# mikelodder7/bls-bn254

Hardware: AMD Instinct MI355X
Metric: BN254 pairings/sec (= BLS verifies/sec) (higher is better)
Workload: dtype int64; 1 GPU; 262144 batched single-sig BLS verifies per GPU (BASELINE configs[1]), unique 32-byte messages, 1024-key pool, 1/64 invalid tuples; key de-duplication + hash-to-G1 + per-key G2 checks and line tables + 2-pair Miller loop + final exp; tuples_per_gpu=262144, tuples_total=262144, key_pool=1024

## Files before the change

### bls-bn254_amd/csrc/fp29.h

```cpp
#pragma once
#include <stdint.h>
#include "bn254_consts.h"

#if defined(__HIPCC__)
#include <hip/hip_runtime.h>
#define BN_HD __host__ __device__
#else
#define BN_HD
#endif
#define BN_INL BN_HD inline __attribute__((always_inline))
#ifdef BN_FORCE_INLINE
#define BN_FUNC BN_INL
#else
#define BN_FUNC BN_HD inline
#endif

#define BN_UNROLL _Pragma("unroll")
#if defined(__HIP_DEVICE_COMPILE__)
#define BN_SCHED_BARRIER __builtin_amdgcn_sched_barrier(0)
#else
#define BN_SCHED_BARRIER ((void)0)
#endif

#ifdef BN_CHECK
#include <cmath>
#include <cstdio>
#include <cstdlib>
#endif

namespace bn {

constexpr int NL = 9;
constexpr int RB = 29;
constexpr int32_t MASK = (1 << RB) - 1;

struct Fp {
  int32_t l[NL];
#ifdef BN_CHECK
  double lo = 0, hi = 0;
  double tlo = 0, thi = 0;
  double vb = 0;
#endif
};

#ifdef BN_CHECK
struct CheckStats { double worst_mul = 0, worst_dot = 0, worst_vb = 0; long muls = 0, sqrs = 0, dots = 0, norms = 0, lcs = 0, lc_terms = 0; };
inline CheckStats& check_stats() { static thread_local CheckStats s; return s; }
inline double mag(const Fp& a) { return std::fmax(std::fabs(a.lo), std::fabs(a.hi)); }
inline double tmag(const Fp& a) { return std::fmax(std::fabs(a.tlo), std::fabs(a.thi)); }
struct CtxStack { const char* name[64]; int line[64]; int n = 0; };
inline CtxStack& ctx_stack() { static thread_local CtxStack s; return s; }
struct CtxGuard {
  CtxGuard(const char* f, int l) { CtxStack& s = ctx_stack(); if (s.n < 64) { s.name[s.n] = f; s.line[s.n] = l; } ++s.n; }
  ~CtxGuard() { --ctx_stack().n; }
};
inline void check_fail(const char* what, double v) {
  std::fprintf(stderr, "BN_CHECK violation: %s (%g)\n  context:", what, v);
  CtxStack& s = ctx_stack();
  for (int i = 0; i < s.n && i < 64; ++i) std::fprintf(stderr, " > %s:%d", s.name[i], s.line[i]);
  std::fprintf(stderr, "\n");
  std::abort();
}
#define BN_CTX ::bn::CtxGuard _bn_ctx_guard(__func__, __LINE__)
inline void check_actual(const Fp& a, const char* where) {
  const double L = 536870912.0;
  for (int i = 0; i < NL; ++i) {
    double v = a.l[i] / L, lo = i == NL - 1 ? a.tlo : a.lo, hi = i == NL - 1 ? a.thi : a.hi;
    if (v < lo - 1e-6 || v > hi + 1e-6) { std::fprintf(stderr, "limb %d = %g outside [%g,%g] at %s\n", i, v, lo, hi, where); check_fail("actual limb outside proven interval", v); }
  }
// ... 473 lines not shown
```

### bls-bn254_amd/csrc/host.hip

```cpp
#include "host_common.h"

extern "C" {

const uint8_t NEG_G2_BYTES[128] = {
  0x19,0x8e,0x93,0x93,0x92,0x0d,0x48,0x3a,0x72,0x60,0xbf,0xb7,0x31,0xfb,0x5d,0x25,0xf1,0xaa,0x49,0x33,0x35,0xa9,0xe7,0x12,0x97,0xe4,0x85,0xb7,0xae,0xf3,0x12,0xc2,
  0x18,0x00,0xde,0xef,0x12,0x1f,0x1e,0x76,0x42,0x6a,0x00,0x66,0x5e,0x5c,0x44,0x79,0x67,0x43,0x22,0xd4,0xf7,0x5e,0xda,0xdd,0x46,0xde,0xbd,0x5c,0xd9,0x92,0xf6,0xed,
  0x27,0x5d,0xc4,0xa2,0x88,0xd1,0xaf,0xb3,0xcb,0xb1,0xac,0x09,0x18,0x75,0x24,0xc7,0xdb,0x36,0x39,0x5d,0xf7,0xbe,0x3b,0x99,0xe6,0x73,0xb1,0x3a,0x07,0x5a,0x65,0xec,
  0x1d,0x9b,0xef,0xcd,0x05,0xa5,0x32,0x3e,0x6d,0xa4,0xd4,0x35,0xf3,0xb6,0x17,0xcd,0xb3,0xaf,0x83,0x28,0x5c,0x2d,0xf7,0x11,0xef,0x39,0xc0,0x15,0x71,0x82,0x7f,0x9d};


const char* blsbn254_strerror(int code) {
  switch (code) {
    case 0: return "ok";
    case 1: return "invalid scalar bytes";
    case 2: return "invalid G1 bytes";
    case 3: return "invalid G2 bytes";
    case 4: return "invalid Gt bytes";
    case BLSBN254_ST_SHORT: return "too few usable partial signatures";
    case BLSBN254_E_ARG: return "invalid argument";
    case BLSBN254_E_HIP: return "HIP runtime error";
    case BLSBN254_E_NOMEM: return "out of device memory";
    case BLSBN254_E_NO_DEVICE: return "no gfx950 device available (there is no CPU fallback)";
    case BLSBN254_E_RCCL: return "RCCL error";
    default: return "unknown error";
// ... 8 lines not shown
  if (hipGetDeviceCount(&count) != hipSuccess || count <= 0 || device < 0 || device >= count) return BLSBN254_E_NO_DEVICE;
  hipDeviceProp_t prop;
  if (hipGetDeviceProperties(&prop, device) != hipSuccess) return BLSBN254_E_NO_DEVICE;
  if (std::strncmp(prop.gcnArchName, "gfx950", 6) != 0) return BLSBN254_E_NO_DEVICE;
  blsbn254_ctx* c = new blsbn254_ctx();
  c->device = device;
  if (const char* e = std::getenv("BLSBN254_CHUNK_LANES")) {
    size_t v = (size_t)std::strtoull(e, nullptr, 10) & ~(size_t)7;
    if (v >= 8 && v <= ((size_t)1 << 23)) c->chunk = v;
  }
  if (hipSetDevice(device) != hipSuccess || hipStreamCreateWithFlags(&c->stream, hipStreamNonBlocking) != hipSuccess) { delete c; return BLSBN254_E_HIP; }
  if (hipStreamCreateWithFlags(&c->stream2, hipStreamNonBlocking) != hipSuccess || hipEventCreateWithFlags(&c->ev_fork, hipEventDisableTiming) != hipSuccess ||
      hipEventCreateWithFlags(&c->ev_join, hipEventDisableTiming) != hipSuccess) { (void)hipStreamDestroy(c->stream); delete c; return BLSBN254_E_HIP; }
  if (getrandom(&c->kd_seed, sizeof c->kd_seed, 0) != (ssize_t)sizeof c->kd_seed) c->kd_seed = 0x5bd1e995u;
  if (const char* e = std::getenv("BLSBN254_AUTO_PREPARE")) c->auto_prepare = std::atoi(e) != 0;
  if (const char* e = std::getenv("BLSBN254_RLC_GROUP")) { long v = std::atol(e); if (v >= 2 && v <= 4096) { c->rlc_group = (size_t)v; c->rlc_group_auto = false; } }
  c->lanes_per_round = (size_t)prop.multiProcessorCount * 256;
  if (const char* e = std::getenv("BLSBN254_RLC_KEY_ROUND")) c->rlc_key_round = std::atoi(e) != 0;
  if (const char* e = std::getenv("BLSBN254_WIDE_FE")) c->wide_fe = std::atoi(e) != 0;
  if (const char* e = std::getenv("BLSBN254_ASYNC_VERIFY")) c->async_verify = std::atoi(e) != 0;
  if (const char* e = std::getenv("BLSBN254_KEY_CACHE")) { long v = std::atol(e); if (v >= 0 && v <= (long)PREP_MAX_KEYS) c->kc.max = (size_t)v; }
  if (const char* e = std::getenv("BLSBN254_QUAD_PREP")) c->quad_prep = std::atoi(e) != 0;
  if (const char* e = std::getenv("BLSBN254_SPLIT_EASY")) c->split_easy = std::atoi(e) != 0;
  c->tri_max = c->lanes_per_round / 4;
  if (const char* e = std::getenv("BLSBN254_TRI_MILLER")) c->tri_miller = std::atoi(e) != 0;
  if (const char* e = std::getenv("BLSBN254_TRI_FE")) c->tri_fe = std::atoi(e) != 0;
  if (const char* e = std::getenv("BLSBN254_TRI_MAX")) { long v = std::atol(e); if (v >= 0 && v <= (1 << 20)) c->tri_max = (size_t)v; }
  if (const char* e = std::getenv("BLSBN254_WIDE_FE_MAX")) { long v = std::atol(e); if (v >= 0 && v <= (1 << 20)) c->wide_fe_max = (size_t)v; }
  *out = c;
  return 0;
}
void blsbn254_ctx_destroy(blsbn254_ctx* c) {
  if (!c) return;
  (void)hipSetDevice(c->device);
  (void)hipStreamSynchronize(c->stream);
  (void)hipStreamSynchronize(c->stream2);
  for (auto& pv : c->pend) if (pv.ev) (void)hipEventDestroy(pv.ev);
  if (c->pend_host) (void)hipHostFree(c->pend_host);
  for (auto& kv : c->prof) for (auto& pr : kv.second.pending) { (void)hipEventDestroy(pr.first); (void)hipEventDestroy(pr.second); }
  (void)hipEventDestroy(c->ev_fork); (void)hipEventDestroy(c->ev_join);
  (void)hipStreamDestroy(c->stream2);
  (void)hipStreamDestroy(c->stream);
  delete c;
}
int blsbn254_ctx_synchronize(blsbn254_ctx* c) {
  if (!c) return BLSBN254_E_ARG;
// ... 101 lines not shown
  HIPCHK(c, hipMemcpyAsync(d, none, 4 * words, hipMemcpyHostToDevice, c->stream));
  return 0;
}
int min_index_read(blsbn254_ctx* c, const int* d, int* out) {
  TRY(download(c, out, d, 4));
  if (*out == NO_INDEX) *out = -1;
  return 0;
}
int first_bad(blsbn254_ctx* c, const uint8_t* d_status, size_t n, uint8_t mask, uint8_t val, int* out) {
  HIPCHK(c, c->misc.reserve(64));
  TRY(min_index_arm(c, (int*)c->misc.p, 1));
  TRY(launch(c, c->stream, "status_reduce", grid_lanes(n), k_status_reduce, d_status, n, mask, val, (int*)c->misc.p));
  return min_index_read(c, (const int*)c->misc.p, out);
}
int read_status(blsbn254_ctx* c, const uint8_t* d_status, int idx, uint8_t* st) { return download(c, st, d_status + idx, 1); }


int run_final_exp(blsbn254_ctx* c, int32_t* f, size_t n, size_t stride, int mode, const uint8_t* flags, const uint8_t* sub_ok,
                         uint8_t* d_bitmap, uint8_t* d_gt, int* d_is_one) {
  CHECK_LANES(c, stride);
  for (DevBuf& b : c->fe) HIPCHK(c, b.reserve(stride * 108 * 4));
  HIPCHK(c, c->fe_slots.reserve(stride * 108 * 4 * 10));
  int32_t* S = (int32_t*)c->fe_slots.p;
  int32_t *X = (int32_t*)c->fe[0].p, *A = (int32_t*)c->fe[1].p, *B = (int32_t*)c->fe[2].p, *C = (int32_t*)c->fe[3].p,
          *B2 = (int32_t*)c->fe[4].p, *D = (int32_t*)c->fe[5].p;
  if (n >= c->lanes_per_round / 2 && c->split_easy) {
    TRY(launch(c, c->stream, "fe_easy_head", grid_lanes(n), k_fe_easy_head, (const int32_t*)f, n, stride, A, B));
    TRY(launch(c, c->stream, "fe_inv4", grid_lanes((n + 3) / 4), k_fe_inv4, B, n, stride));
    TRY(launch(c, c->stream, "fe_easy_tail", grid_lanes(n), k_fe_easy_tail, (const int32_t*)f, f, n, stride, (const int32_t*)A, (const int32_t*)B));
  } else {
    TRY(launch(c, c->stream, "fe_easy", grid_lanes(n), k_fe_easy, (const int32_t*)f, f, n, stride));
  }
  if (c->wide_fe && n <= c->wide_fe_max) {
    uint8_t* one = nullptr;
    if (mode == 0) { HIPCHK(c, c->fe_wide_one.reserve(n)); one = (uint8_t*)c->fe_wide_one.p; }
    TRY(launch(c, c->stream, "fe_hard_wide", grid_wide(n), k_fe_hard_wide, (const int32_t*)f, n, stride, flags, sub_ok, one, d_gt, d_is_one, mode));
    if (mode == 0) TRY(launch(c, c->stream, "pack_bitmap", grid_lanes(n), k_pack_bitmap, (const uint8_t*)one, n, d_bitmap));
    return 0;
  }
  if (n <= c->tri_max && c->tri_fe) {
    HIPCHK(c, c->tri_vals.reserve(n * TRI_VALUE_LIMBS * 4));
    uint8_t* one = nullptr;
    if (mode == 0) { HIPCHK(c, c->fe_wide_one.reserve(n)); one = (uint8_t*)c->fe_wide_one.p; }
    TRY(launch(c, c->stream, "fe_tri_hard", grid_tri(n), k_fe_tri_hard, (const int32_t*)f, n, stride, (int32_t*)c->tri_vals.p, flags, sub_ok, one, d_gt, d_is_one, mode));
    if (mode == 0) TRY(launch(c, c->stream, "pack_bitmap", grid_lanes(n), k_pack_bitmap, (const uint8_t*)one, n, d_bitmap));
    return 0;
  }
  TRY(launch(c, c->stream, "fe_expx_h1", grid_lanes(n), k_fe_expx_h1, (const int32_t*)f, S, n, stride, A, B));
  TRY(launch(c, c->stream, "fe_expx_h2", grid_lanes(n), k_fe_expx_h2, (const int32_t*)B, S, n, stride, B, C, B2, D));
  TRY(launch(c, c->stream, "fe_expx", grid_lanes(n), k_fe_expx, (const int32_t*)D, X, S, n, stride));
  TRY(launch(c, c->stream, "fe_h3", grid_lanes(n), k_fe_h3, (const int32_t*)f, (const int32_t*)A, (const int32_t*)C, (const int32_t*)B2, (const int32_t*)X, S, n, stride,
             flags, sub_ok, d_bitmap, d_gt, d_is_one, mode));
  return 0;
}

int miller_to_ws(blsbn254_ctx* c, const uint8_t* d_g1, const uint8_t* d_g2, size_t n) {
  CHECK_LANES(c, n);
  HIPCHK(c, c->f_ws.reserve(n * 108 * 4));
  HIPCHK(c, c->status.reserve(n));
  if (c->wide_fe && n <= c->wide_fe_max / 2) {
    TRY(launch(c, c->stream, "miller_wide_1", grid_wide(n), k_miller_wide_1, d_g1, d_g2, n, (int32_t*)c->f_ws.p, n, (uint8_t*)c->status.p));
  } else if (n <= c->tri_max && c->tri_miller) {
    TRY(launch(c, c->stream, "miller_tri_1", grid_tri(n), k_miller_tri_1, d_g1, d_g2, n, (int32_t*)c->f_ws.p, n, (uint8_t*)c->status.p));
  } else {
    TRY(launch(c, c->stream, "miller_1", grid_lanes(n), k_miller_1, d_g1, d_g2, n, (int32_t*)c->f_ws.p, n, (uint8_t*)c->status.p));
  }
  return 0;
}
int decode_status_rc(blsbn254_ctx* c, const uint8_t* d_status, size_t n) {
  int bad;
  int rc = first_bad(c, d_status, n, 3, 3, &bad);
  if (rc) return rc;
  if (bad < 0) return 0;
  uint8_t st; rc = read_status(c, d_status, bad, &st);
  if (rc) return rc;
// ... 130 lines not shown
```

### bls-bn254_amd/csrc/host_common.h

```cpp
#pragma once
#include <hip/hip_runtime.h>
#include <sys/random.h>
#include <cstdio>
#include <cstdlib>
#include <cstring>
#include <algorithm>
#include <map>
#include <string>
#include <vector>

#include "sha256.h"
#include "lane_ops.h"
#include "kernels.h"
#include "key_cache.h"
#include "seg_plan.h"
#include "keyset_agg_plan.h"
#include "../../include/blsbn254.h"

using namespace bn;

#define BNH __attribute__((visibility("hidden")))

struct BNH DevBuf {
  void* p = nullptr; size_t cap = 0;
// ... 82 lines not shown
  uint32_t kd_seed = 0;
  bool auto_prepare = true;
  uint64_t stat_prepared_chunks = 0, stat_exact_chunks = 0, stat_grouped_aggregates = 0, stat_pairwise_aggregates = 0;
  DevBuf q_ws;
  DevBuf th_x, th_num, th_den, th_glv, th_part, th_part2;
  DevBuf fe_wide_one;
  bool wide_fe = true;
  size_t tri_max = 16384;
  bool tri_miller = true, tri_fe = true;
  DevBuf tri_vals;
  struct PendingVerify {
    bool active = false; const uint8_t *d_pks = nullptr, *d_msgs = nullptr, *d_sigs = nullptr; const uint64_t* d_off = nullptr;
    size_t n = 0; uint8_t* d_bitmap = nullptr; uint8_t dst[256]; size_t dst_len = 0; hipEvent_t ev = nullptr;
  } pend[4];
  int pend_head = 0, pend_count = 0;
  uint32_t* pend_host = nullptr;
  DevBuf pend_dev;
  size_t u_hint = 0;
  size_t u_max_seen = 0;
  bool async_verify = true;
  uint64_t stat_async_chunks = 0, stat_async_reruns = 0;
  bool quad_prep = true;
  bool split_easy = true;
  size_t wide_fe_max = 2048;
  DevBuf gs_items, gs_items_ok, gs_sum, gs_sum_ok, gs_pk;
  SegWs gs;
  DevBuf fe_slots;
  uint8_t dst_host[256];
  int dst_host_len = -1;
  size_t chunk = (size_t)1 << 22;
  MsmWs msm;
  PcWs pc;
  ThbWs thb;
  AgbWs agb;
  TdlWs tdl;
  TcWs tc;
  KsetWs kset;
  KaggWs kagg;
  uint64_t stat_kset[4] = {0, 0, 0, 0};
  uint64_t stat_kagg[4] = {0, 0, 0, 0};
  uint64_t stat_tc[4] = {0, 0, 0, 0};
  uint64_t stat_tdl[4] = {0, 0, 0, 0};
  uint64_t stat_agb[4] = {0, 0, 0, 0};
  uint64_t stat_thb[3] = {0, 0, 0};
  int msm_window = 0;
  uint64_t stat_msm[4] = {0, 0, 0, 0};
  bool profiling = false;
  std::map<std::string, ProfEntry> prof;
  std::string last_error;
// ... 152 lines not shown
```

### bls-bn254_amd/csrc/k_fe_easy.hip

```cpp
#include "lane_ops.h"
#include "kernels.h"
using namespace bn;

BN_KERNEL k_fe_easy(const int32_t* in, int32_t* out, size_t n, size_t stride) {
  size_t i = (size_t)blockIdx.x * blockDim.x + threadIdx.x;
  if (i >= n) return;
  fp12_store_limbs(out + i, stride, fe_easy(fp12_load_limbs(in + i, stride)));
}
BN_KERNEL k_fe_easy_head(const int32_t* in, size_t n, size_t stride, int32_t* head, int32_t* nu) {
  size_t i = (size_t)blockIdx.x * blockDim.x + threadIdx.x;
  if (i >= n) return;
  const FeEasyHead h = fe_easy_head(fp12_load_limbs(in + i, stride));
  fp2_store_limbs(head + i, stride, h.c0); fp2_store_limbs(head + 18 * stride + i, stride, h.c1);
  fp2_store_limbs(head + 36 * stride + i, stride, h.c2); fp2_store_limbs(head + 54 * stride + i, stride, h.nrm);
  store_fp(nu + i, stride, h.nu);
}
BN_KERNEL k_fe_inv4(int32_t* nu, size_t n, size_t stride) {
  const size_t q = (n + 3) / 4;
  size_t j = (size_t)blockIdx.x * blockDim.x + threadIdx.x;
  if (j >= q) return;
  Fp x[4];
  for (int t = 0; t < 4; ++t) { const size_t i = j + (size_t)t * q; x[t] = i < n ? load_fp(nu + i, stride) : fp_one(); }
  fp_inv4(x);
  for (int t = 0; t < 4; ++t) { const size_t i = j + (size_t)t * q; if (i < n) store_fp(nu + i, stride, x[t]); }
}
```

### bls-bn254_amd/csrc/k_fe_expx_tail.hip

```cpp
#include "lane_ops.h"
#include "kernels.h"
using namespace bn;

BN_KERNEL k_fe_expx_h1(const int32_t* in, int32_t* slots, size_t n, size_t stride, int32_t* a_out, int32_t* b_out) {
  __shared__ int32_t park_lds[108 * 256];
  size_t i = (size_t)blockIdx.x * blockDim.x + threadIdx.x;
  if (i >= n) return;
  const uint32_t l4 = (uint32_t)i * 4u;
  const Ws park = {park_lds, 256, threadIdx.x * 4u, false};
  Fp12 r = cyclotomic_exp_x_chain(fp12_load_limbs(in + i, stride), Ws{slots, stride, l4, true}, &park);
  fe_h1_tail(r, Ws{a_out, stride, l4, true}, Ws{b_out, stride, l4, true}, &park);
}
BN_KERNEL k_fe_expx_h2(const int32_t* in, int32_t* slots, size_t n, size_t stride, int32_t* b_in, int32_t* c_out, int32_t* b2_out, int32_t* d2_out) {
  __shared__ int32_t park_lds[108 * 256];
  size_t i = (size_t)blockIdx.x * blockDim.x + threadIdx.x;
  if (i >= n) return;
  const uint32_t l4 = (uint32_t)i * 4u;
  const Ws park = {park_lds, 256, threadIdx.x * 4u, false};
  Fp12 r = cyclotomic_exp_x_chain(fp12_load_limbs(in + i, stride), Ws{slots, stride, l4, true}, &park);
  fe_h2_tail(r, Ws{b_in, stride, l4, true}, Ws{c_out, stride, l4, true}, Ws{b2_out, stride, l4, true}, Ws{d2_out, stride, l4, true}, &park);
}
```

### bls-bn254_amd/csrc/k_fe_h3.hip

```cpp
#include "lane_ops.h"
#include "kernels.h"
using namespace bn;


BN_KERNEL k_fe_h3(const int32_t* t, const int32_t* a, const int32_t* c, const int32_t* b2, const int32_t* x0, int32_t* tmp, size_t n, size_t stride,
                  const uint8_t* flags, const uint8_t* sub_ok, uint8_t* bitmap, uint8_t* gt_bytes, int* is_one, int mode) {
  __shared__ int32_t park_lds[108 * 256];
  const uint32_t i = blockIdx.x * blockDim.x + threadIdx.x;
  bool bit = false;
  if (i < n) {
    const uint32_t l4 = i * 4u;
    const Ws src[5] = {{const_cast<int32_t*>(t), stride, l4, true}, {const_cast<int32_t*>(a), stride, l4, true}, {const_cast<int32_t*>(c), stride, l4, true},
                       {const_cast<int32_t*>(b2), stride, l4, true}, {const_cast<int32_t*>(x0), stride, l4, true}};
    const Ws park = {park_lds, 256, threadIdx.x * 4u, false};
    Fp12 r = fe_h3_loop(src, Ws{tmp, stride, l4, true}, &park);
    if (mode == 0) bit = fp12_is_one(r) & (flags[i] == (FLAG_SIG_OK | FLAG_PK_OK)) & (sub_ok[i] != 0);
    else if (mode == 3) *is_one = fp12_is_one(r) ? 1 : 0;
    else if (mode == 4) gt_bytes[i] = fp12_is_one(r) ? 1 : 0;
    else fp12_to_be(gt_bytes + 384 * (size_t)i, r);
  }
  if (mode == 0) write_ballot(bitmap, n, i, bit);
}
```

### bls-bn254_amd/csrc/kernels.h

```cpp
#pragma once
#include <hip/hip_runtime.h>
#include <stddef.h>
#include <stdint.h>

#ifndef BN_WAVES_PER_SIMD
#define BN_WAVES_PER_SIMD 1
#endif
#define BN_KERNEL __global__ void __launch_bounds__(256, BN_WAVES_PER_SIMD)

#if defined(__HIPCC__)
__device__ inline void write_ballot(uint8_t* bitmap, size_t n, size_t i, bool bit) {
  unsigned long long m = __ballot(bit);
  unsigned lane = threadIdx.x & 63;
  size_t base = (i - lane) >> 3;
  size_t nbytes = (n + 7) >> 3;
  if (lane < 8 && base + lane < nbytes) bitmap[base + lane] = (uint8_t)(m >> (8 * lane));
}
#endif

BN_KERNEL k_hash_to_g1(const uint8_t* msgs, const uint64_t* off, size_t n, const uint8_t* dst, uint32_t dst_len,
                       int32_t* h_ws, size_t h_stride, uint8_t* out_bytes, int mode);
BN_KERNEL k_hash_to_g2(const uint8_t* msgs, const uint64_t* off, size_t n, const uint8_t* dst, uint32_t dst_len,
                       uint8_t* out_bytes, int ro);
BN_KERNEL k_g1_check(const uint8_t* g1, size_t n, uint8_t* bitmap);
BN_KERNEL k_g2_check(const uint8_t* g2, size_t n, uint8_t* ok_bytes, uint8_t* bitmap);
BN_KERNEL k_miller_1(const uint8_t* g1, const uint8_t* g2, size_t n, int32_t* f_ws, size_t f_stride, uint8_t* status);
BN_KERNEL k_miller_hpk(const int32_t* h_ws, const uint8_t* pks, size_t n, int32_t* f_ws, size_t f_stride, uint8_t* flags);
BN_KERNEL k_miller_hpk2(const int32_t* h_ws, const uint8_t* pks, size_t n, int32_t* q_ws, int32_t* f_ws, size_t f_stride, uint8_t* flags);
BN_KERNEL k_miller_hpk2p(const int32_t* h_ws, size_t h_stride, const uint32_t* kid, const int32_t* table, const uint8_t* key_ok, size_t n,
                         int32_t* f_ws, size_t f_stride, uint8_t* flags, const uint8_t* skip);
BN_KERNEL k_miller_hpk1p(const int32_t* h_ws, size_t h_stride, const uint32_t* kid, const int32_t* table, const uint8_t* key_ok, size_t n,
                         int32_t* f_ws, size_t f_stride, uint8_t* flags, const uint8_t* skip);
BN_KERNEL k_g1_to_ws_batch(const uint8_t* g1, size_t n, int32_t* h_ws, uint8_t* status);
BN_KERNEL k_g1_to_ws(const uint8_t* g1, int32_t* h_ws, size_t slot, size_t stride, uint8_t* ok);
BN_KERNEL k_miller_verify(const uint8_t* pks, const uint8_t* sigs, const int32_t* h_ws, size_t n, int32_t* f_ws, uint8_t* flags);
BN_KERNEL k_fe_easy(const int32_t* in, int32_t* out, size_t n, size_t stride);
BN_KERNEL k_fe_easy_head(const int32_t* in, size_t n, size_t stride, int32_t* head, int32_t* nu);
BN_KERNEL k_fe_inv4(int32_t* nu, size_t n, size_t stride);
BN_KERNEL k_fe_easy_tail(const int32_t* in, int32_t* out, size_t n, size_t stride, const int32_t* head, const int32_t* nu);
BN_KERNEL k_fe_expx(const int32_t* in, int32_t* out, int32_t* slots, size_t n, size_t stride);
BN_KERNEL k_fe_expx_h1(const int32_t* in, int32_t* slots, size_t n, size_t stride, int32_t* a_out, int32_t* b_out);
BN_KERNEL k_fe_expx_h2(const int32_t* in, int32_t* slots, size_t n, size_t stride, int32_t* b_in, int32_t* c_out, int32_t* b2_out, int32_t* d2_out);
BN_KERNEL k_fe_h3(const int32_t* t, const int32_t* a, const int32_t* c, const int32_t* b2, const int32_t* x0, int32_t* tmp, size_t n, size_t stride,
                  const uint8_t* flags, const uint8_t* sub_ok, uint8_t* bitmap, uint8_t* gt_bytes, int* is_one, int mode);
__global__ void __launch_bounds__(128) k_miller_wide_prepared(const uint32_t* perm, const uint32_t* kid, const uint8_t* sigs, const int32_t* h_ws, size_t h_stride,
                                                             const int32_t* table, const uint8_t* key_ok, size_t n, int32_t* f_ws, uint8_t* flags);
__global__ void __launch_bounds__(128) k_miller_wide_1p(const int32_t* h_ws, size_t h_stride, const uint32_t* kid, const int32_t* table, const uint8_t* key_ok, size_t n,
                                                       int32_t* f_ws, size_t f_stride, uint8_t* flags, const uint8_t* skip);
__global__ void __launch_bounds__(128) k_miller_wide_1(const uint8_t* g1, const uint8_t* g2, size_t n, int32_t* f_ws, size_t f_stride, uint8_t* status);
__global__ void __launch_bounds__(128) k_fe_hard_wide(const int32_t* t_ws, size_t n, size_t stride, const uint8_t* flags, const uint8_t* sub_ok,
                                                     uint8_t* one, uint8_t* gt_bytes, int* is_one, int mode);
BN_KERNEL k_fp12_from_bytes(const uint8_t* in, size_t n, int32_t* f_ws, size_t f_stride, uint8_t* status);
BN_KERNEL k_fp12_to_bytes(const int32_t* f_ws, size_t n, size_t stride, uint8_t* out);
BN_KERNEL k_fp12_mul_pairs(const int32_t* in, size_t n_in, size_t in_stride, int32_t* out, size_t out_stride);
BN_KERNEL k_g1_load(const uint8_t* g1, size_t n, int32_t* ws, uint8_t* status);
BN_KERNEL k_g1_add_pairs(const int32_t* in, size_t n_in, size_t in_stride, int32_t* out, size_t out_stride);
BN_KERNEL k_g1_to_bytes(const int32_t* ws, size_t stride, uint8_t* out);
BN_KERNEL k_sign(const uint8_t* sks, const uint8_t* msgs, const uint64_t* off, size_t n, const uint8_t* dst, uint32_t dst_len,
                 uint8_t* sigs, uint8_t* status);
BN_KERNEL k_sk_to_pk(const uint8_t* sks, size_t n, uint8_t* pks, uint8_t* status);
BN_KERNEL k_g1_mul(const uint8_t* g1, const uint8_t* scalars, size_t n, uint8_t* out, uint8_t* status);
BN_KERNEL k_g2_mul(const uint8_t* g2, const uint8_t* scalars, size_t n, uint8_t* out, uint8_t* status);
BN_KERNEL k_g2_load(const uint8_t* g2, size_t n, int32_t* ws, uint8_t* ok);
BN_KERNEL k_g2_seg_sum(const int32_t* in_ws, size_t in_stride, const uint8_t* ok_in, const uint32_t* chunk_start, const uint32_t* chunk_len, size_t m,
                       int32_t* out_ws, size_t out_stride, uint8_t* ok_out);
BN_KERNEL k_pair_ok(const uint8_t* g1, const uint8_t* g2, size_t n, uint8_t* ok);
BN_KERNEL k_fp12_seg_prod(const int32_t* in_ws, size_t in_stride, const uint8_t* ok_in, const uint32_t* chunk_start, const uint32_t* chunk_len,
// ... 105 lines not shown
```

### bls-bn254_amd/csrc/pairing.h

```cpp
#pragma once
#include "curve.h"

namespace bn {

struct G2J { Fp2 x, y, z; };
struct Line { Fp2 c0, c1, c2; };

BN_FUNC Line doubling_step(G2J& r) {
  BN_CTX;
  Fp2 tmp0 = fp2_sqr(r.x);
  Fp2 tmp1 = fp2_sqr(r.y);
  Fp2 tmp2 = fp2_sqr(tmp1);
  Fp2 s3 = fp2_sqr(fp2_norm(fp2_add(tmp1, r.x)));
  Fp2 tmp3 = f_lc3<2, -2, -2>(s3, tmp0, tmp2);
  Fp2 tmp4 = f_lc2<3, 0>(tmp0, tmp0);
  Fp2 tmp6 = fp2_norm(fp2_add(r.x, tmp4));
  Fp2 tmp5 = fp2_sqr(tmp4);
  Fp2 zsq = fp2_sqr(r.z);
  Fp2 nx = f_lc2<1, -2>(tmp5, tmp3);
  Fp2 nz = fp2_norm(fp2_sub(fp2_sub(fp2_sqr(fp2_norm(fp2_add(r.z, r.y))), tmp1), zsq));
  Fp2 ny = f_lc2<1, -8>(fp2_mul(fp2_sub(tmp3, nx), tmp4), tmp2);
  Line l;
  l.c1 = f_lc2<-2, 0>(fp2_mul(tmp4, zsq), zsq);
  Fp2 s6 = fp2_sub(fp2_sub(fp2_sqr(tmp6), tmp0), tmp5);
// ... 325 lines not shown
  BN_CTX;
  Fp6 s0 = fp6_sqr(a.c0), s1 = fp6_sqr(a.c1);
  Fp6 d = {fp2_sub_mul_xi(s0.c0, s1.c2), fp2_norm(fp2_sub(s0.c1, s1.c0)), fp2_norm(fp2_sub(s0.c2, s1.c1))};
  Fp2 q0 = fp2_sqr(d.c0), q1 = fp2_sqr(d.c1), q2 = fp2_sqr(d.c2);
  Fp2 m01 = fp2_mul(d.c0, d.c1), m02 = fp2_mul(d.c0, d.c2), m12 = fp2_mul(d.c1, d.c2);
  FeEasyHead h;
  h.c0 = fp2_sub_mul_xi(q0, m12);
  h.c1 = fp2_norm(fp2_sub(fp2_mul_xi(q2), m01));
  h.c2 = fp2_norm(fp2_sub(q1, m02));
  Fp2 u = fp2_add(fp2_mul(d.c2, h.c1), fp2_mul(d.c1, h.c2));
  h.nrm = fp2_add_mul_xi(fp2_mul(d.c0, h.c0), u);
  h.nu = fp_dot2(h.nrm.c0, h.nrm.c0, h.nrm.c1, h.nrm.c1);
  return h;
}
BN_FUNC Fp12 fe_easy_tail(const Fp12& a, const FeEasyHead& h, const Fp& nu_inv) {
  BN_CTX;
  Fp2 ti = {fp_mul(h.nrm.c0, nu_inv), fp_mul(fp_neg(h.nrm.c1), nu_inv)};
  Fp6 t6 = {fp2_mul(h.c0, ti), fp2_mul(h.c1, ti), fp2_mul(h.c2, ti)};
  Fp12 inv = {fp6_mul(a.c0, t6), fp6_norm(fp6_neg(fp6_mul(a.c1, t6)))};
  Fp12 t = fp12_mul(fp12_conj(a), inv);
  return fp12_mul(fp12_frob<2>(t), t);
}
template <bool POW_FALLBACK = true>
BN_FUNC bool fp_inv4(Fp x[4]) {
  BN_CTX;
  bool z[4];
  Fp v[4], pre[4];
  for (int i = 0; i < 4; ++i) { z[i] = fp_is_zero(x[i]); v[i] = fp_select(z[i], fp_one(), fp_norm(x[i])); }
  pre[0] = v[0];
  for (int i = 1; i < 4; ++i) pre[i] = fp_mul(pre[i - 1], v[i]);
  bool done = true;
  Fp inv = POW_FALLBACK ? fp_inv(pre[3]) : fp_inv_divsteps(pre[3], done);
  for (int i = 3; i >= 1; --i) {
    Fp r = fp_mul(inv, pre[i - 1]);
    inv = fp_mul(inv, v[i]);
    x[i] = fp_select(z[i], fp_zero(), r);
  }
  x[0] = fp_select(z[0], fp_zero(), inv);
  return done;
}
BN_FUNC void fe_h1(const Fp12& x0, Fp12& a, Fp12& b) {
  a = fp12_cyclotomic_sqr(fp12_conj(x0));
  Fp12 a2 = fp12_cyclotomic_sqr(a);
  b = fp12_mul(a, a2);
}
BN_FUNC void fe_h2(const Fp12& x0, const Fp12& b, Fp12& c, Fp12& b2, Fp12& d2) {
  c = fp12_conj(x0);
  b2 = fp12_mul(c, fp12_conj(b));
  d2 = fp12_cyclotomic_sqr(c);
}
BN_FUNC Fp12 fe_h3(const Fp12& t, const Fp12& a, const Fp12& c, const Fp12& b2, const Fp12& x0) {
  Fp12 e = fp12_mul(b2, x0);
  Fp12 d = fp12_mul(a, e);
  Fp12 l0 = fp12_mul(t, fp12_mul(c, e));
  Fp12 r = fp12_mul(l0, fp12_frob<1>(d));
  r = fp12_mul(r, fp12_frob<2>(e));
  Fp12 l3 = fp12_mul(fp12_conj(t), d);
  return fp12_mul(r, fp12_frob<3>(l3));
}
BN_FUNC Fp12 final_exponentiation(const Fp12& f) {
  Fp12 t = fe_easy(f), a, b, c, b2, d2;
// ... 45 lines not shown
  BN_CTX;
  return {{fp2_load_limbs(w), fp2_load_limbs(ws_at(w, 18)), fp2_load_limbs(ws_at(w, 36))},
          {fp2_load_limbs(ws_at(w, 54)), fp2_load_limbs(ws_at(w, 72)), fp2_load_limbs(ws_at(w, 90))}};
}
BN_FUNC void fp12_store_limbs(int32_t* out, size_t stride, const Fp12& a) {
  BN_CTX;
  fp2_store_limbs(out, stride, a.c0.c0); fp2_store_limbs(out + 18 * stride, stride, a.c0.c1);
  fp2_store_limbs(out + 36 * stride, stride, a.c0.c2); fp2_store_limbs(out + 54 * stride, stride, a.c1.c0);
  fp2_store_limbs(out + 72 * stride, stride, a.c1.c1); fp2_store_limbs(out + 90 * stride, stride, a.c1.c2);
}
BN_INL Fp2 fp2_load_limbs(const int32_t* in, size_t stride) {
  Fp2 c;
  BN_UNROLL for (int k = 0; k < NL; ++k) { c.c0.l[k] = in[(size_t)k * stride]; c.c1.l[k] = in[(size_t)(9 + k) * stride]; }
  BN_TRK(set_trk(c.c0, 0, 1, 0, 0.006, 1); set_trk(c.c1, 0, 1, 0, 0.006, 1);)
  return c;
}
BN_FUNC Fp12 fp12_load_limbs(const int32_t* in, size_t stride) {
  BN_CTX;
  return {{fp2_load_limbs(in, stride), fp2_load_limbs(in + 18 * stride, stride), fp2_load_limbs(in + 36 * stride, stride)},
          {fp2_load_limbs(in + 54 * stride, stride), fp2_load_limbs(in + 72 * stride, stride), fp2_load_limbs(in + 90 * stride, stride)}};
}

struct H3Op { int8_t pre, mul, post; };
BN_FUNC Fp12 fe_h3_loop(const Ws* src, const Ws& tmp, const Ws* park) {
  const H3Op prog[8] = {{1, 4, 1}, {0, 1, 2}, {2, 0, 3}, {3, 2, 0}, {0, 0, 0}, {0, 7, 0}, {0, 6, 0}, {0, 8, 0}};
  Fp12 r = fp12_one();
  for (int k = 0; k < 8; ++k) {
    const H3Op op = prog[k];
    if (op.pre == 1) r = fp12_load_mem(src[3]);
    else if (op.pre == 2) r = fp12_conj(r);
    else if (op.pre == 3) r = fp12_load_mem(tmp);
    const int m = op.mul;
    const Ws b = m == 0 ? src[0] : m == 1 ? src[1] : m == 2 ? src[2] : m == 4 ? src[4] : ws_at(tmp, 108 * (size_t)(m - 5));
    r = fp12_mul_mem(r, b, park);
    if (op.post == 1) { fp12_store_mem(tmp, r); fp12_store_mem(ws_at(tmp, 108), fp12_frob<2>(r)); }
    else if (op.post == 2) fp12_store_mem(ws_at(tmp, 216), fp12_frob<1>(r));
    else if (op.post == 3) fp12_store_mem(ws_at(tmp, 324), fp12_frob<3>(fp12_conj(r)));
    BN_MEM_FENCE;
  }
  return r;
}

BN_FUNC void fe_h1_tail(const Fp12& x0, const Ws& a_out, const Ws& b_out, const Ws* park) {
  Fp12 a = fp12_cyclotomic_sqr(fp12_conj(x0));
  fp12_store_mem(a_out, a);
  BN_MEM_FENCE;
  fp12_store_mem(b_out, fp12_mul_mem(fp12_cyclotomic_sqr(a), a_out, park));
}
BN_FUNC void fe_h2_tail(const Fp12& x0, const Ws& b_in, const Ws& c_out, const Ws& b2_out, const Ws& d2_out, const Ws* park) {
  fp12_store_mem(c_out, fp12_conj(x0));
  BN_MEM_FENCE;
  fp12_store_mem(b2_out, fp12_conj(fp12_mul_mem(x0, b_in, park)));
  BN_MEM_FENCE;
  fp12_store_mem(d2_out, fp12_cyclotomic_sqr(fp12_load_mem(c_out)));
}

BN_INL void line_store_limbs(const Ws& w, const Line& l) { fp2_store_limbs(w, l.c0); fp2_store_limbs(ws_at(w, 18), l.c1); fp2_store_limbs(ws_at(w, 36), l.c2); }
BN_INL Line line_load_limbs(const Ws& w) { return {fp2_load_limbs(w), fp2_load_limbs(ws_at(w, 18)), fp2_load_limbs(ws_at(w, 36))}; }
BN_FUNC void g2_prepare_lines(const G2A& q, const Ws& out) {
  BN_CTX;
  G2J T = {q.x, q.y, fp2_one()};
  Fp2 nqy = fp2_norm(fp2_neg(q.y));
  int ti = 0;
// ... 248 lines not shown
```

### bls-bn254_amd/csrc/tower.h

```cpp
#pragma once
#include "fp29.h"

namespace bn {

struct Fp2 { Fp c0, c1; };
struct Fp6 { Fp2 c0, c1, c2; };
struct Fp12 { Fp6 c0, c1; };

BN_INL Fp2 fp2_add(const Fp2& a, const Fp2& b) { return {fp_add(a.c0, b.c0), fp_add(a.c1, b.c1)}; }
BN_INL Fp2 fp2_sub(const Fp2& a, const Fp2& b) { return {fp_sub(a.c0, b.c0), fp_sub(a.c1, b.c1)}; }
BN_INL Fp2 fp2_neg(const Fp2& a) { return {fp_neg(a.c0), fp_neg(a.c1)}; }
BN_INL Fp2 fp2_dbl(const Fp2& a) { return {fp_dbl(a.c0), fp_dbl(a.c1)}; }
BN_INL Fp2 fp2_conj(const Fp2& a) { return {a.c0, fp_neg(a.c1)}; }
BN_INL Fp2 fp2_norm(const Fp2& a) { return {fp_norm(a.c0), fp_norm(a.c1)}; }
BN_INL Fp2 fp2_zero() { return {fp_zero(), fp_zero()}; }
BN_INL Fp2 fp2_one() { return {fp_one(), fp_zero()}; }
BN_INL Fp2 fp2_const(const int32_t (&c)[2 * NL]) {
  Fp2 r;
  BN_UNROLL for (int i = 0; i < NL; ++i) { r.c0.l[i] = c[i]; r.c1.l[i] = c[NL + i]; }
  BN_TRK(set_trk(r.c0, 0, 1, 0, 0.006, 1); set_trk(r.c1, 0, 1, 0, 0.006, 1);)
  return r;
}
BN_INL Fp2 fp2_from_limbs(const int32_t* c) { return {fp_from_limbs(c), fp_from_limbs(c + NL)}; }
BN_INL Fp2 fp2_select(bool cond, const Fp2& a, const Fp2& b) { return {fp_select(cond, a.c0, b.c0), fp_select(cond, a.c1, b.c1)}; }
// ... 128 lines not shown
#endif
BN_INL Fp fp_load_mem(const Ws& w) {
  Fp r;
  BN_UNROLL for (int k = 0; k < NL; ++k) r.l[k] = ws_load(w, k);
  BN_TRK(ParkTrk pt; { std::lock_guard<std::mutex> g(park_mutex()); auto it = park_trk().find(ws_addr(w, 0));
           if (it == park_trk().end()) check_fail("fp_load_mem of an address never stored", 0); pt = it->second; }
         set_trk(r, pt.lo, pt.hi, pt.tlo, pt.thi, pt.vb);)
  return r;
}
BN_INL void fp_store_mem(const Ws& w, const Fp& a) {
  BN_TRK(if (a.lo < -4e-6 || a.hi > 1.0 + 4e-6) check_fail("fp_store_mem needs a normalised value", mag(a));
         { std::lock_guard<std::mutex> g(park_mutex()); park_trk()[ws_addr(w, 0)] = ParkTrk{a.lo, a.hi, a.tlo, a.thi, a.vb}; })
  BN_UNROLL for (int k = 0; k < NL; ++k) ws_store(w, k, a.l[k]);
}
BN_INL Fp2 fp2_load_mem(const Ws& w) { return {fp_load_mem(w), fp_load_mem(ws_at(w, 9))}; }
BN_INL Fp6 fp6_load_mem(const Ws& w) { return {fp2_load_mem(w), fp2_load_mem(ws_at(w, 18)), fp2_load_mem(ws_at(w, 36))}; }
BN_INL void fp2_store_mem(const Ws& w, const Fp2& a) { fp_store_mem(w, a.c0); fp_store_mem(ws_at(w, 9), a.c1); }
BN_INL void fp6_store_mem(const Ws& w, const Fp6& a) {
  fp2_store_mem(w, a.c0); fp2_store_mem(ws_at(w, 18), a.c1); fp2_store_mem(ws_at(w, 36), a.c2);
}
BN_INL void fp12_store_mem(const Ws& w, const Fp12& a) { fp6_store_mem(w, a.c0); fp6_store_mem(ws_at(w, 54), a.c1); }
BN_INL Fp12 fp12_load_mem(const Ws& w) { return {fp6_load_mem(w), fp6_load_mem(ws_at(w, 54))}; }
BN_FUNC Fp12 fp12_mul_mem(const Fp12& a, const Ws& b, const Ws* park = nullptr) {
  Fp6 v0, v1, w;
  if (park) {
    Fp6 b0 = fp6_load_mem(b), b1 = fp6_load_mem(ws_at(b, 54));
    fp6_store_mem(ws_at(*park, 54), fp6_norm(fp6_sub(b1, b0)));
    v0 = fp6_mul(a.c0, b0);
    fp6_store_mem(*park, v0);
    BN_MEM_FENCE;
    v1 = fp6_mul(a.c1, b1);
    BN_MEM_FENCE;
    w = fp6_mul(fp6_norm(fp6_sub(a.c0, a.c1)), fp6_load_mem(ws_at(*park, 54)));
    v0 = fp6_load_mem(*park);
  } else {
    { Fp6 b0 = fp6_load_mem(b); v0 = fp6_mul(a.c0, b0); }
    BN_MEM_FENCE;
    { Fp6 b1 = fp6_load_mem(ws_at(b, 54)); v1 = fp6_mul(a.c1, b1); }
    BN_MEM_FENCE;
    { Fp6 b0 = fp6_load_mem(b), b1 = fp6_load_mem(ws_at(b, 54));
      w = fp6_mul(fp6_norm(fp6_sub(a.c0, a.c1)), fp6_norm(fp6_sub(b1, b0))); }
  }
  return {fp6_add_mul_v(v0, v1), fp6_norm(fp6_add(fp6_add(w, v0), v1))};
}
BN_FUNC Fp12 fp12_sqr(const Fp12& a) {
  Fp6 ab = fp6_mul(a.c0, a.c1);
// ... 58 lines not shown
BN_INL Fp2 cyc_c1(const Fp4Sq& q, const Fp2& z) {
  return {fp_lc4<3, -3, -3, 2>(q.s.c0, q.ta.c0, q.tb.c0, z.c0), fp_lc4<3, -3, -3, 2>(q.s.c1, q.ta.c1, q.tb.c1, z.c1)};
}
BN_FUNC Fp12 fp12_cyclotomic_sqr(const Fp12& f) {
  BN_CTX;
  Fp2 z0 = f.c0.c0, z4 = f.c0.c1, z3 = f.c0.c2, z2 = f.c1.c0, z1 = f.c1.c1, z5 = f.c1.c2;
  Fp4Sq q01 = fp4_sq_raw(z0, z1);
  Fp2 r0 = cyc_c0(q01, z0), r1 = cyc_c1(q01, z1);
  Fp4Sq q23 = fp4_sq_raw(z2, z3);
  Fp2 r4 = cyc_c0(q23, z4), r5 = cyc_c1(q23, z5);
  Fp4Sq q45 = fp4_sq_raw(z4, z5);
  Fp2 r3 = cyc_c0(q45, z3);
  Fp2 t5 = {fp_lc4<1, -1, -1, 0, true>(q45.s.c0, q45.ta.c0, q45.tb.c0, q45.s.c0), fp_lc4<1, -1, -1, 0, true>(q45.s.c1, q45.ta.c1, q45.tb.c1, q45.s.c1)};
  Fp2 r2 = {fp_lc3<27, -3, 2>(t5.c0, t5.c1, z2.c0), fp_lc3<3, 27, 2>(t5.c0, t5.c1, z2.c1)};
  return {{r0, r4, r3}, {r2, r1, r5}};
}
BN_INL bool fp12_is_one(const Fp12& a) {
  bool z = fp_is_zero(fp_sub(a.c0.c0.c0, fp_one()));
  z &= fp_is_zero(a.c0.c0.c1);
  z &= fp2_is_zero(a.c0.c1) & fp2_is_zero(a.c0.c2);
  z &= fp2_is_zero(a.c1.c0) & fp2_is_zero(a.c1.c1) & fp2_is_zero(a.c1.c2);
  return z;
}

}
```

Baseline: 8.009 million verifies/s.

## Fuse final expx into h3 kernel and replace last Fp12 mul with conjugate-equality check

For verdict modes, the final-exponentiation tail now ends one Fp12 multiplication early and decides r == 1 by checking whether the partial product equals the conjugate (inverse in the cyclotomic subgroup) of the stored last factor. A separate invertibility flag from the easy-part inversion is carried through so a zero Miller output is not accepted. The last exp-by-x chain is also fused into the h3 kernel, so x0 stays in registers and one launch plus a global round-trip are dropped. In exchange the fused kernel holds more live state, which may raise register pressure, and correctness now relies on the new inverse-equality test and the zero flag.

```diff
diff --git a/bls-bn254_amd/csrc/fp29.h b/bls-bn254_amd/csrc/fp29.h
--- a/bls-bn254_amd/csrc/fp29.h
+++ b/bls-bn254_amd/csrc/fp29.h
@@ -44,7 +44,7 @@
 };
 
 #ifdef BN_CHECK
-struct CheckStats { double worst_mul = 0, worst_dot = 0, worst_vb = 0; long muls = 0, sqrs = 0, dots = 0, norms = 0, lcs = 0, lc_terms = 0; };
+struct CheckStats { double worst_mul = 0, worst_dot = 0, worst_vb = 0; long muls = 0, sqrs = 0, dots = 0, norms = 0, lcs = 0, lc_terms = 0, fp12_mul_mems = 0; };
 inline CheckStats& check_stats() { static thread_local CheckStats s; return s; }
 inline double mag(const Fp& a) { return std::fmax(std::fabs(a.lo), std::fabs(a.hi)); }
 inline double tmag(const Fp& a) { return std::fmax(std::fabs(a.tlo), std::fabs(a.thi)); }
diff --git a/bls-bn254_amd/csrc/host.hip b/bls-bn254_amd/csrc/host.hip
--- a/bls-bn254_amd/csrc/host.hip
+++ b/bls-bn254_amd/csrc/host.hip
@@ -54,6 +54,7 @@
   if (const char* e = std::getenv("BLSBN254_KEY_CACHE")) { long v = std::atol(e); if (v >= 0 && v <= (long)PREP_MAX_KEYS) c->kc.max = (size_t)v; }
   if (const char* e = std::getenv("BLSBN254_QUAD_PREP")) c->quad_prep = std::atoi(e) != 0;
   if (const char* e = std::getenv("BLSBN254_SPLIT_EASY")) c->split_easy = std::atoi(e) != 0;
+  if (const char* e = std::getenv("BLSBN254_FUSE_H3")) c->fuse_h3 = std::atoi(e) != 0;
   c->tri_max = c->lanes_per_round / 4;
   if (const char* e = std::getenv("BLSBN254_TRI_MILLER")) c->tri_miller = std::atoi(e) != 0;
   if (const char* e = std::getenv("BLSBN254_TRI_FE")) c->tri_fe = std::atoi(e) != 0;
@@ -201,14 +202,16 @@
   for (DevBuf& b : c->fe) HIPCHK(c, b.reserve(stride * 108 * 4));
   HIPCHK(c, c->fe_slots.reserve(stride * 108 * 4 * 10));
   int32_t* S = (int32_t*)c->fe_slots.p;
+  HIPCHK(c, c->fe_inv_ok.reserve(n));
+  uint8_t* inv_ok = (uint8_t*)c->fe_inv_ok.p;
   int32_t *X = (int32_t*)c->fe[0].p, *A = (int32_t*)c->fe[1].p, *B = (int32_t*)c->fe[2].p, *C = (int32_t*)c->fe[3].p,
           *B2 = (int32_t*)c->fe[4].p, *D = (int32_t*)c->fe[5].p;
   if (n >= c->lanes_per_round / 2 && c->split_easy) {
     TRY(launch(c, c->stream, "fe_easy_head", grid_lanes(n), k_fe_easy_head, (const int32_t*)f, n, stride, A, B));
-    TRY(launch(c, c->stream, "fe_inv4", grid_lanes((n + 3) / 4), k_fe_inv4, B, n, stride));
+    TRY(launch(c, c->stream, "fe_inv4", grid_lanes((n + 3) / 4), k_fe_inv4, B, n, stride, inv_ok));
     TRY(launch(c, c->stream, "fe_easy_tail", grid_lanes(n), k_fe_easy_tail, (const int32_t*)f, f, n, stride, (const int32_t*)A, (const int32_t*)B));
   } else {
-    TRY(launch(c, c->stream, "fe_easy", grid_lanes(n), k_fe_easy, (const int32_t*)f, f, n, stride));
+    TRY(launch(c, c->stream, "fe_easy", grid_lanes(n), k_fe_easy, (const int32_t*)f, f, n, stride, inv_ok));
   }
   if (c->wide_fe && n <= c->wide_fe_max) {
     uint8_t* one = nullptr;
@@ -227,9 +230,14 @@
   }
   TRY(launch(c, c->stream, "fe_expx_h1", grid_lanes(n), k_fe_expx_h1, (const int32_t*)f, S, n, stride, A, B));
   TRY(launch(c, c->stream, "fe_expx_h2", grid_lanes(n), k_fe_expx_h2, (const int32_t*)B, S, n, stride, B, C, B2, D));
+  if ((mode == 0 || mode == 3 || mode == 4) && c->fuse_h3) {
+    TRY(launch(c, c->stream, "fe_expx_h3", grid_lanes(n), k_fe_expx_h3, (const int32_t*)D, S, n, stride, (const int32_t*)f, (const int32_t*)A, (const int32_t*)C,
+               (const int32_t*)B2, (const uint8_t*)inv_ok, flags, sub_ok, d_bitmap, d_gt, d_is_one, mode));
+    return 0;
+  }
   TRY(launch(c, c->stream, "fe_expx", grid_lanes(n), k_fe_expx, (const int32_t*)D, X, S, n, stride));
   TRY(launch(c, c->stream, "fe_h3", grid_lanes(n), k_fe_h3, (const int32_t*)f, (const int32_t*)A, (const int32_t*)C, (const int32_t*)B2, (const int32_t*)X, S, n, stride,
-             flags, sub_ok, d_bitmap, d_gt, d_is_one, mode));
+             (const uint8_t*)inv_ok, flags, sub_ok, d_bitmap, d_gt, d_is_one, mode));
   return 0;
 }
 
diff --git a/bls-bn254_amd/csrc/host_common.h b/bls-bn254_amd/csrc/host_common.h
--- a/bls-bn254_amd/csrc/host_common.h
+++ b/bls-bn254_amd/csrc/host_common.h
@@ -128,9 +128,11 @@
   uint64_t stat_async_chunks = 0, stat_async_reruns = 0;
   bool quad_prep = true;
   bool split_easy = true;
+  bool fuse_h3 = true;
   size_t wide_fe_max = 2048;
   DevBuf gs_items, gs_items_ok, gs_sum, gs_sum_ok, gs_pk;
   SegWs gs;
+  DevBuf fe_inv_ok;
   DevBuf fe_slots;
   uint8_t dst_host[256];
   int dst_host_len = -1;
diff --git a/bls-bn254_amd/csrc/k_fe_easy.hip b/bls-bn254_amd/csrc/k_fe_easy.hip
--- a/bls-bn254_amd/csrc/k_fe_easy.hip
+++ b/bls-bn254_amd/csrc/k_fe_easy.hip
@@ -2,10 +2,12 @@
 #include "kernels.h"
 using namespace bn;
 
-BN_KERNEL k_fe_easy(const int32_t* in, int32_t* out, size_t n, size_t stride) {
+BN_KERNEL k_fe_easy(const int32_t* in, int32_t* out, size_t n, size_t stride, uint8_t* inv_ok) {
   size_t i = (size_t)blockIdx.x * blockDim.x + threadIdx.x;
   if (i >= n) return;
-  fp12_store_limbs(out + i, stride, fe_easy(fp12_load_limbs(in + i, stride)));
+  const Fp12 f = fp12_load_limbs(in + i, stride);
+  inv_ok[i] = fp12_is_zero(f) ? 0 : 1;
+  fp12_store_limbs(out + i, stride, fe_easy(f));
 }
 BN_KERNEL k_fe_easy_head(const int32_t* in, size_t n, size_t stride, int32_t* head, int32_t* nu) {
   size_t i = (size_t)blockIdx.x * blockDim.x + threadIdx.x;
@@ -15,12 +17,13 @@
   fp2_store_limbs(head + 36 * stride + i, stride, h.c2); fp2_store_limbs(head + 54 * stride + i, stride, h.nrm);
   store_fp(nu + i, stride, h.nu);
 }
-BN_KERNEL k_fe_inv4(int32_t* nu, size_t n, size_t stride) {
+BN_KERNEL k_fe_inv4(int32_t* nu, size_t n, size_t stride, uint8_t* inv_ok) {
   const size_t q = (n + 3) / 4;
   size_t j = (size_t)blockIdx.x * blockDim.x + threadIdx.x;
   if (j >= q) return;
   Fp x[4];
   for (int t = 0; t < 4; ++t) { const size_t i = j + (size_t)t * q; x[t] = i < n ? load_fp(nu + i, stride) : fp_one(); }
-  fp_inv4(x);
-  for (int t = 0; t < 4; ++t) { const size_t i = j + (size_t)t * q; if (i < n) store_fp(nu + i, stride, x[t]); }
+  bool z[4];
+  fp_inv4(x, z);
+  for (int t = 0; t < 4; ++t) { const size_t i = j + (size_t)t * q; if (i < n) { store_fp(nu + i, stride, x[t]); inv_ok[i] = z[t] ? 0 : 1; } }
 }
diff --git a/bls-bn254_amd/csrc/k_fe_expx_tail.hip b/bls-bn254_amd/csrc/k_fe_expx_tail.hip
--- a/bls-bn254_amd/csrc/k_fe_expx_tail.hip
+++ b/bls-bn254_amd/csrc/k_fe_expx_tail.hip
@@ -20,3 +20,23 @@
   Fp12 r = cyclotomic_exp_x_chain(fp12_load_limbs(in + i, stride), Ws{slots, stride, l4, true}, &park);
   fe_h2_tail(r, Ws{b_in, stride, l4, true}, Ws{c_out, stride, l4, true}, Ws{b2_out, stride, l4, true}, Ws{d2_out, stride, l4, true}, &park);
 }
+BN_KERNEL k_fe_expx_h3(const int32_t* in, int32_t* slots, size_t n, size_t stride, const int32_t* t, const int32_t* a, const int32_t* c, const int32_t* b2,
+                       const uint8_t* inv_ok, const uint8_t* flags, const uint8_t* sub_ok, uint8_t* bitmap, uint8_t* out_bytes, int* is_one, int mode) {
+  __shared__ int32_t park_lds[108 * 256];
+  const uint32_t i = blockIdx.x * blockDim.x + threadIdx.x;
+  bool bit = false;
+  if (i < n) {
+    const uint32_t l4 = i * 4u;
+    const Ws park = {park_lds, 256, threadIdx.x * 4u, false};
+    const Ws sw = {slots, stride, l4, true};
+    const Fp12 x0 = cyclotomic_exp_x_chain(fp12_load_limbs(in + i, stride), sw, &park);
+    const Ws src[4] = {{const_cast<int32_t*>(t), stride, l4, true}, {const_cast<int32_t*>(a), stride, l4, true}, {const_cast<int32_t*>(c), stride, l4, true},
+                       {const_cast<int32_t*>(b2), stride, l4, true}};
+    const Fp12 r = fe_h3_loop<true>(src, sw, &park, H3_VERDICT_OPS, &x0);
+    const bool one = fe_h3_is_one(r, sw, inv_ok[i] != 0);
+    if (mode == 0) bit = one & (flags[i] == (FLAG_SIG_OK | FLAG_PK_OK)) & (sub_ok[i] != 0);
+    else if (mode == 3) *is_one = one ? 1 : 0;
+    else out_bytes[i] = one ? 1 : 0;
+  }
+  if (mode == 0) write_ballot(bitmap, n, i, bit);
+}
diff --git a/bls-bn254_amd/csrc/k_fe_h3.hip b/bls-bn254_amd/csrc/k_fe_h3.hip
--- a/bls-bn254_amd/csrc/k_fe_h3.hip
+++ b/bls-bn254_amd/csrc/k_fe_h3.hip
@@ -4,7 +4,7 @@
 
 
 BN_KERNEL k_fe_h3(const int32_t* t, const int32_t* a, const int32_t* c, const int32_t* b2, const int32_t* x0, int32_t* tmp, size_t n, size_t stride,
-                  const uint8_t* flags, const uint8_t* sub_ok, uint8_t* bitmap, uint8_t* gt_bytes, int* is_one, int mode) {
+                  const uint8_t* inv_ok, const uint8_t* flags, const uint8_t* sub_ok, uint8_t* bitmap, uint8_t* gt_bytes, int* is_one, int mode) {
   __shared__ int32_t park_lds[108 * 256];
   const uint32_t i = blockIdx.x * blockDim.x + threadIdx.x;
   bool bit = false;
@@ -13,11 +13,15 @@
     const Ws src[5] = {{const_cast<int32_t*>(t), stride, l4, true}, {const_cast<int32_t*>(a), stride, l4, true}, {const_cast<int32_t*>(c), stride, l4, true},
                        {const_cast<int32_t*>(b2), stride, l4, true}, {const_cast<int32_t*>(x0), stride, l4, true}};
     const Ws park = {park_lds, 256, threadIdx.x * 4u, false};
-    Fp12 r = fe_h3_loop(src, Ws{tmp, stride, l4, true}, &park);
-    if (mode == 0) bit = fp12_is_one(r) & (flags[i] == (FLAG_SIG_OK | FLAG_PK_OK)) & (sub_ok[i] != 0);
-    else if (mode == 3) *is_one = fp12_is_one(r) ? 1 : 0;
-    else if (mode == 4) gt_bytes[i] = fp12_is_one(r) ? 1 : 0;
-    else fp12_to_be(gt_bytes + 384 * (size_t)i, r);
+    const bool verdict = mode == 0 || mode == 3 || mode == 4;
+    const Ws tw = {tmp, stride, l4, true};
+    Fp12 r = fe_h3_loop(src, tw, &park, verdict ? H3_VERDICT_OPS : H3_GT_OPS);
+    if (verdict) {
+      const bool one = fe_h3_is_one(r, tw, inv_ok[i] != 0);
+      if (mode == 0) bit = one & (flags[i] == (FLAG_SIG_OK | FLAG_PK_OK)) & (sub_ok[i] != 0);
+      else if (mode == 3) *is_one = one ? 1 : 0;
+      else gt_bytes[i] = one ? 1 : 0;
+    } else fp12_to_be(gt_bytes + 384 * (size_t)i, r);
   }
   if (mode == 0) write_ballot(bitmap, n, i, bit);
 }
diff --git a/bls-bn254_amd/csrc/kernels.h b/bls-bn254_amd/csrc/kernels.h
--- a/bls-bn254_amd/csrc/kernels.h
+++ b/bls-bn254_amd/csrc/kernels.h
@@ -34,15 +34,17 @@
 BN_KERNEL k_g1_to_ws_batch(const uint8_t* g1, size_t n, int32_t* h_ws, uint8_t* status);
 BN_KERNEL k_g1_to_ws(const uint8_t* g1, int32_t* h_ws, size_t slot, size_t stride, uint8_t* ok);
 BN_KERNEL k_miller_verify(const uint8_t* pks, const uint8_t* sigs, const int32_t* h_ws, size_t n, int32_t* f_ws, uint8_t* flags);
-BN_KERNEL k_fe_easy(const int32_t* in, int32_t* out, size_t n, size_t stride);
+BN_KERNEL k_fe_easy(const int32_t* in, int32_t* out, size_t n, size_t stride, uint8_t* inv_ok);
 BN_KERNEL k_fe_easy_head(const int32_t* in, size_t n, size_t stride, int32_t* head, int32_t* nu);
-BN_KERNEL k_fe_inv4(int32_t* nu, size_t n, size_t stride);
+BN_KERNEL k_fe_inv4(int32_t* nu, size_t n, size_t stride, uint8_t* inv_ok);
 BN_KERNEL k_fe_easy_tail(const int32_t* in, int32_t* out, size_t n, size_t stride, const int32_t* head, const int32_t* nu);
 BN_KERNEL k_fe_expx(const int32_t* in, int32_t* out, int32_t* slots, size_t n, size_t stride);
 BN_KERNEL k_fe_expx_h1(const int32_t* in, int32_t* slots, size_t n, size_t stride, int32_t* a_out, int32_t* b_out);
 BN_KERNEL k_fe_expx_h2(const int32_t* in, int32_t* slots, size_t n, size_t stride, int32_t* b_in, int32_t* c_out, int32_t* b2_out, int32_t* d2_out);
+BN_KERNEL k_fe_expx_h3(const int32_t* in, int32_t* slots, size_t n, size_t stride, const int32_t* t, const int32_t* a, const int32_t* c, const int32_t* b2,
+                       const uint8_t* inv_ok, const uint8_t* flags, const uint8_t* sub_ok, uint8_t* bitmap, uint8_t* out_bytes, int* is_one, int mode);
 BN_KERNEL k_fe_h3(const int32_t* t, const int32_t* a, const int32_t* c, const int32_t* b2, const int32_t* x0, int32_t* tmp, size_t n, size_t stride,
-                  const uint8_t* flags, const uint8_t* sub_ok, uint8_t* bitmap, uint8_t* gt_bytes, int* is_one, int mode);
+                  const uint8_t* inv_ok, const uint8_t* flags, const uint8_t* sub_ok, uint8_t* bitmap, uint8_t* gt_bytes, int* is_one, int mode);
 __global__ void __launch_bounds__(128) k_miller_wide_prepared(const uint32_t* perm, const uint32_t* kid, const uint8_t* sigs, const int32_t* h_ws, size_t h_stride,
                                                              const int32_t* table, const uint8_t* key_ok, size_t n, int32_t* f_ws, uint8_t* flags);
 __global__ void __launch_bounds__(128) k_miller_wide_1p(const int32_t* h_ws, size_t h_stride, const uint32_t* kid, const int32_t* table, const uint8_t* key_ok, size_t n,
diff --git a/bls-bn254_amd/csrc/pairing.h b/bls-bn254_amd/csrc/pairing.h
--- a/bls-bn254_amd/csrc/pairing.h
+++ b/bls-bn254_amd/csrc/pairing.h
@@ -371,7 +371,7 @@
   return fp12_mul(fp12_frob<2>(t), t);
 }
 template <bool POW_FALLBACK = true>
-BN_FUNC bool fp_inv4(Fp x[4]) {
+BN_FUNC bool fp_inv4(Fp x[4], bool* was_zero = nullptr) {
   BN_CTX;
   bool z[4];
   Fp v[4], pre[4];
@@ -386,6 +386,7 @@
     x[i] = fp_select(z[i], fp_zero(), r);
   }
   x[0] = fp_select(z[0], fp_zero(), inv);
+  if (was_zero) for (int i = 0; i < 4; ++i) was_zero[i] = z[i];
   return done;
 }
 BN_FUNC void fe_h1(const Fp12& x0, Fp12& a, Fp12& b) {
@@ -477,16 +478,18 @@
 }
 
 struct H3Op { int8_t pre, mul, post; };
-BN_FUNC Fp12 fe_h3_loop(const Ws* src, const Ws& tmp, const Ws* park) {
-  const H3Op prog[8] = {{1, 4, 1}, {0, 1, 2}, {2, 0, 3}, {3, 2, 0}, {0, 0, 0}, {0, 7, 0}, {0, 6, 0}, {0, 8, 0}};
-  Fp12 r = fp12_one();
-  for (int k = 0; k < 8; ++k) {
+constexpr int H3_GT_OPS = 8, H3_VERDICT_OPS = 7;
+template <bool X0_REG = false>
+BN_FUNC Fp12 fe_h3_loop(const Ws* src, const Ws& tmp, const Ws* park, int nops = H3_GT_OPS, const Fp12* x0 = nullptr) {
+  const H3Op prog[8] = {{X0_REG ? 0 : 1, X0_REG ? 3 : 4, 1}, {0, 1, 2}, {2, 0, 3}, {3, 2, 0}, {0, 0, 0}, {0, 7, 0}, {0, 6, 0}, {0, 8, 0}};
+  Fp12 r = X0_REG ? *x0 : fp12_one();
+  for (int k = 0; k < nops; ++k) {
     const H3Op op = prog[k];
     if (op.pre == 1) r = fp12_load_mem(src[3]);
     else if (op.pre == 2) r = fp12_conj(r);
     else if (op.pre == 3) r = fp12_load_mem(tmp);
     const int m = op.mul;
-    const Ws b = m == 0 ? src[0] : m == 1 ? src[1] : m == 2 ? src[2] : m == 4 ? src[4] : ws_at(tmp, 108 * (size_t)(m - 5));
+    const Ws b = m == 0 ? src[0] : m == 1 ? src[1] : m == 2 ? src[2] : m == 3 ? src[3] : m == 4 ? src[X0_REG ? 3 : 4] : ws_at(tmp, 108 * (size_t)(m - 5));
     r = fp12_mul_mem(r, b, park);
     if (op.post == 1) { fp12_store_mem(tmp, r); fp12_store_mem(ws_at(tmp, 108), fp12_frob<2>(r)); }
     else if (op.post == 2) fp12_store_mem(ws_at(tmp, 216), fp12_frob<1>(r));
@@ -494,6 +497,9 @@
     BN_MEM_FENCE;
   }
   return r;
+}
+BN_FUNC bool fe_h3_is_one(const Fp12& R, const Ws& tmp, bool f_invertible) {
+  return fp12_eq_conj(R, fp12_load_mem(ws_at(tmp, 324))) & f_invertible;
 }
 
 BN_FUNC void fe_h1_tail(const Fp12& x0, const Ws& a_out, const Ws& b_out, const Ws* park) {
diff --git a/bls-bn254_amd/csrc/tower.h b/bls-bn254_amd/csrc/tower.h
--- a/bls-bn254_amd/csrc/tower.h
+++ b/bls-bn254_amd/csrc/tower.h
@@ -174,6 +174,7 @@
 BN_INL void fp12_store_mem(const Ws& w, const Fp12& a) { fp6_store_mem(w, a.c0); fp6_store_mem(ws_at(w, 54), a.c1); }
 BN_INL Fp12 fp12_load_mem(const Ws& w) { return {fp6_load_mem(w), fp6_load_mem(ws_at(w, 54))}; }
 BN_FUNC Fp12 fp12_mul_mem(const Fp12& a, const Ws& b, const Ws* park = nullptr) {
+  BN_TRK(++check_stats().fp12_mul_mems;)
   Fp6 v0, v1, w;
   if (park) {
     Fp6 b0 = fp6_load_mem(b), b1 = fp6_load_mem(ws_at(b, 54));
@@ -278,5 +279,16 @@
   z &= fp2_is_zero(a.c1.c0) & fp2_is_zero(a.c1.c1) & fp2_is_zero(a.c1.c2);
   return z;
 }
-
-}
+BN_INL bool fp12_is_zero(const Fp12& a) {
+  bool z = fp2_is_zero(a.c0.c0) & fp2_is_zero(a.c0.c1) & fp2_is_zero(a.c0.c2);
+  z &= fp2_is_zero(a.c1.c0) & fp2_is_zero(a.c1.c1) & fp2_is_zero(a.c1.c2);
+  return z;
+}
+BN_INL bool fp2_eq_neg(const Fp2& a, const Fp2& b) { return fp2_is_zero(fp2_add(a, b)); }
+BN_INL bool fp12_eq_conj(const Fp12& a, const Fp12& s) {
+  bool z = fp2_eq(a.c0.c0, s.c0.c0) & fp2_eq(a.c0.c1, s.c0.c1) & fp2_eq(a.c0.c2, s.c0.c2);
+  z &= fp2_eq_neg(a.c1.c0, s.c1.c0) & fp2_eq_neg(a.c1.c1, s.c1.c1) & fp2_eq_neg(a.c1.c2, s.c1.c2);
+  return z;
+}
+
+}
```

New measurement: 8.071 million verifies/s (median of 6 runs). Within noise of the previous version (+0.8%).
